# 123456jack/decision-making-and-path-planning

Measured on AMD Instinct MI355X. Metric: planning ticks/sec (batched scenes), 512x512 grid, higher is better.
Workload: dtype f64; 1 GPU; BASELINE configs[1]: 1024 scenes/GPU, 512x512 grid, 64 static obstacles; scenes_per_gpu=1024, global_scenes=1024, grid=512, obstacles=64, parallelism=scene-sharded x1, RCCL scatter/gather outside the timed region, algorithmic_bytes_per_tick=276644

## Files before the change

### decision-making-and-path-planning_amd/csrc/dmpp_hip.hip

```cpp
#include <hip/hip_runtime.h>
#include <cstddef>
#include <cstdio>
#include <cstring>
#include <cmath>
#include <string>
#include <cstdlib>
#include <vector>
#include <new>
#include <algorithm>
#include "../../include/dmpp_planner.h"
#include "kernels_r.hpp"
#include "kernels_a.hpp"
#include "kernels_rt.hpp"
#include "kernels_ep.hpp"
#include "kernels_es.hpp"
#include "kernels_g.hpp"
#include "kernels_sc.hpp"
#include "kernels_el.hpp"
#include "kernels_f.hpp"
#include "kernels_t.hpp"
#include "kernels_op.hpp"
#include "search_budget.hpp"

namespace {
// ... 1992 lines not shown
    if (h->rec_last.tick != T) {
        { int r = join_all(h); if (r) return r; }
        hipEvent_t e = get_sync_event(h);
        if (!e) return fail(PP_ERR_HIP, "event creation failed");
        HIP_TRY(hipEventRecord(e, h->stream));
        TickRec rec = { T, h->in_cur, e, nullptr };
        h->inflight.push_back(rec); h->rec_last = rec;
    }
    const TickRec& R = h->rec_last;
    if (h->done_tick[slot] != T) { h->done_tick[slot] = T; h->done_g[slot].forget(); h->done_p[slot].forget(); }
    const bool want_plan = plan || result || show;
    PendingFetch f{};
    f.tick = T; f.slot = slot; f.n = (size_t)n; f.ev_front = R.ev_front; f.ev_tail = R.ev_tail;
    if (want_plan) { f.plan_dst = plan; f.res_dst = result; f.show_dst = show; f.plan_src = h->d_plan; f.plan_set = h->plan_cur; }
    if (grid) { f.grid_dst = grid; f.grid_src = h->d_gout[h->gout_set]; f.grid_set = h->gout_set; }
    bool joined = false;
    for (PendingFetch& g : h->fetches) if (g.tick == T) {
        if (want_plan && !g.plan_dst && !g.res_dst && !g.show_dst) { g.plan_dst = f.plan_dst; g.res_dst = f.res_dst; g.show_dst = f.show_dst; g.plan_src = f.plan_src; g.plan_set = f.plan_set; g.plan_issued = false; joined = true; }
        if (grid && !g.grid_dst) { g.grid_dst = f.grid_dst; g.grid_src = f.grid_src; g.grid_set = f.grid_set; g.grid_issued = false; joined = true; }
    }
    if (!joined) h->fetches.push_back(f);
    { int r = pump_fetches(h); if (r) return r; }
    if (tick_id) *tick_id = T;
    return PP_OK;
}

int pp_fetch_async(pp_handle h, PlanOut* plan, GridOut* grid, long long* tick_id) { return fetch_async(h, plan, nullptr, nullptr, grid, tick_id); }
int pp_fetch_published_async(pp_handle h, PlanningOut* result, PlanningStatus* show, GridOut* grid, long long* tick_id)
{ return fetch_async(h, nullptr, result, show, grid, tick_id); }

long long pp_tick_id(pp_handle h) { return h ? h->tick_seq : -1; }

int pp_wait_tick(pp_handle h, long long tick_id, int* n_poisoned)
{
    if (!h) return fail(PP_ERR_ARG, "null handle");
    if (n_poisoned) *n_poisoned = 0;
    if (tick_id <= 0 || tick_id > h->tick_seq) return fail(PP_ERR_ARG, "pp_wait_tick: no such tick");
    const int slot = (int)(tick_id % kDone);
    if (!h->streaming || h->done_tick[slot] != tick_id)
        return fail(PP_ERR_ARG, "pp_wait_tick: no pp_fetch_async was issued for that tick (or more than " + std::to_string(kDone) + " ticks ago)");
    HIP_TRY(hipSetDevice(h->device));
    { int r = flush_group(h); if (r) return r; }
    { int r = pump_fetches(h, tick_id); if (r) return r; }
    PP_TRY(h->done_p[slot].host_wait());
    PP_TRY(h->done_g[slot].host_wait());
    const int bad = (int)reinterpret_cast<volatile int32_t*>(h->h_bad.get())[slot];
    if (n_poisoned) *n_poisoned = bad;
    if (bad) return fail(PP_ERR_ARG, "tick " + std::to_string(tick_id) + ": " + std::to_string(bad) + " scene(s) of its update had a slice outside its pool (or a road / lane outside the map) and ran with empty inputs");
    return PP_OK;
}

int pp_tick_io(pp_handle h, PpSceneIo* io)
{
    if (!h || !io) return fail(PP_ERR_ARG, "null argument");
    if (h->n_scenes != 1) return fail(PP_ERR_STATE, "pp_tick_io moves ONE resident scene (pp_set_scenes with n_scenes = 1 comes first: its lane pool stays)");
    if ((io->want & PP_IO_WANT_GRID) && !h->cfg.grid_stage) return fail(PP_ERR_STATE, "PP_IO_WANT_GRID: the handle's configuration has the grid stage off");
    HIP_TRY(hipSetDevice(h->device));
    const int max_obs = std::min(PP_IO_MAX_OBS, h->caps.max_obs_total), max_ref = std::min(DMPP_MAX_REFPATH, h->caps.max_ref_pts_total);
    { int r = flush_group(h); if (r) return r; }
    PP_TRY(h->score.ego.wait(h->stream));
    h->in_staged = -1; h->rollout.staged_by_advance = false;
    hipLaunchKernelGGL(dmpp::k_io_in, dim3(1), dim3(dmpp::kBlock), 0, h->stream, io, max_obs, max_ref, h->n_lane_pts, h->d_in, h->d_state, h->d_obs, h->d_ref);
    HIP_TRY(hipGetLastError());
    h->n_obs_total = std::min(std::max((int)io->n_obs, 0), max_obs); h->have_motion = false;
    h->n_ref_pts = std::max(h->n_ref_pts, max_ref);
    note_current_set(h);
    { int r = pp_plan_tick(h); if (r) return r; }
    if (h->last_piped) { int r = join_all(h); if (r) return r; }
    hipLaunchKernelGGL(dmpp::k_io_out, dim3(1), dim3(dmpp::kBlock), 0, h->stream, io, (int)io->want, h->d_plan, h->d_state,
                       h->cfg.grid_stage ? h->d_gout[h->gout_set] : nullptr, h->d_dec_ref);
    HIP_TRY(hipGetLastError());
    HIP_TRY(hipStreamSynchronize(h->stream));
    if (reinterpret_cast<volatile int32_t*>(&io->status)[0]) return fail(PP_ERR_ARG, "pp_tick_io: a lane slice of io->in lies outside the resident lane pool (the scene ran with empty lanes)");
    return PP_OK;
}

#ifdef DMPP_DEBUG_SEARCH
int pp_debug_score_counters(int* out8, int reset)
{
    HIP_TRY(hipMemcpyFromSymbol(out8, HIP_SYMBOL(dmpp::g_dbg_score), 8 * sizeof(int)));
    if (reset) { int z[8] = { 0 }; HIP_TRY(hipMemcpyToSymbol(HIP_SYMBOL(dmpp::g_dbg_score), z, sizeof(z))); }
    return PP_OK;
}
#endif

void* pp_host_alloc(size_t bytes)
{
    void* p = nullptr;
    if (hipHostMalloc(&p, bytes ? bytes : 1, hipHostMallocDefault) != hipSuccess) { (void)hipGetLastError(); g_err = "hipHostMalloc failed"; return nullptr; }
    return p;
}
void pp_host_free(void* p) { if (p) (void)hipHostFree(p); }
int pp_host_register(void* p, size_t bytes)
{
    if (!p || !bytes) return fail(PP_ERR_ARG, "null argument");
    HIP_TRY(hipHostRegister(p, bytes, hipHostRegisterDefault));
    return PP_OK;
}
int pp_host_unregister(void* p) { if (!p) return PP_OK; HIP_TRY(hipHostUnregister(p)); return PP_OK; }

static int need_scratch(pp_handle h, size_t bytes)
{
    if (bytes <= h->d_scratch.capacity()) return PP_OK;
    HIP_TRY(hipStreamSynchronize(h->stream));
    return h->d_scratch.reserve(bytes);
}
static size_t al256(size_t v) { return (v + 255) & ~(size_t)255; }

int pp_search_obstacle_batch(pp_handle h, int nq, const GlobalPoint2D* paths, const int32_t* path_off, const ObPoint* obs,
                             const int32_t* obs_off, const double* lat_lo, const double* lat_hi, Path_Obs* out)
{
    if (!h || !paths || !path_off || !obs_off || !lat_lo || !lat_hi || !out) return fail(PP_ERR_ARG, "null argument");
    if (nq <= 0) return PP_OK;
    HIP_TRY(hipSetDevice(h->device));
    const int np = path_off[nq], no = obs_off[nq];
    for (int q = 0; q < nq; q++) if (path_off[q + 1] - path_off[q] > dmpp::kSoMaxPts) return fail(PP_ERR_CAPACITY, "a path longer than 2048 points");
    size_t o_paths = 0, o_poff = o_paths + al256((size_t)np * sizeof(GlobalPoint2D)), o_obs = o_poff + al256((size_t)(nq + 1) * 4),
           o_ooff = o_obs + al256((size_t)no * sizeof(ObPoint)), o_lo = o_ooff + al256((size_t)(nq + 1) * 4),
           o_hi = o_lo + al256((size_t)nq * 8), o_out = o_hi + al256((size_t)nq * 8), total = o_out + al256((size_t)nq * sizeof(Path_Obs));
    int r = need_scratch(h, total); if (r) return r;
    char* d = (char*)h->d_scratch;
    if (np) HIP_TRY(hipMemcpyAsync(d + o_paths, paths, (size_t)np * sizeof(GlobalPoint2D), hipMemcpyDefault, h->stream));
    HIP_TRY(hipMemcpyAsync(d + o_poff, path_off, (size_t)(nq + 1) * 4, hipMemcpyDefault, h->stream));
    if (no && obs) HIP_TRY(hipMemcpyAsync(d + o_obs, obs, (size_t)no * sizeof(ObPoint), hipMemcpyDefault, h->stream));
    HIP_TRY(hipMemcpyAsync(d + o_ooff, obs_off, (size_t)(nq + 1) * 4, hipMemcpyDefault, h->stream));
    HIP_TRY(hipMemcpyAsync(d + o_lo, lat_lo, (size_t)nq * 8, hipMemcpyDefault, h->stream));
    HIP_TRY(hipMemcpyAsync(d + o_hi, lat_hi, (size_t)nq * 8, hipMemcpyDefault, h->stream));
    hipLaunchKernelGGL(dmpp::k_search_obstacle_batch, dim3(nq), dim3(DMPP_WAVE), 0, h->stream, h->cfg, nq,
                       (const GlobalPoint2D*)(d + o_paths), (const int32_t*)(d + o_poff), (const ObPoint*)(d + o_obs),
                       (const int32_t*)(d + o_ooff), (const double*)(d + o_lo), (const double*)(d + o_hi), (Path_Obs*)(d + o_out));
    HIP_TRY(hipGetLastError());
    HIP_TRY(hipMemcpyAsync(out, d + o_out, (size_t)nq * sizeof(Path_Obs), hipMemcpyDefault, h->stream));
    HIP_TRY(hipStreamSynchronize(h->stream));
    return PP_OK;
}

int pp_geom_batch(pp_handle h, int op, int n, const GlobalPoint2D* a, const GlobalPoint2D* b, const GlobalPoint2D* c3, double* out)
{
    if (!h || !a || !out || op < 0 || op > 5) return fail(PP_ERR_ARG, "bad argument");
    if (((op <= 1 || op == 3) && !b) || (op == 0 && !c3)) return fail(PP_ERR_ARG, "missing operand");
    if (n <= 0) return PP_OK;
    HIP_TRY(hipSetDevice(h->device));
    const size_t pb = al256((size_t)n * sizeof(GlobalPoint2D));
    int r = need_scratch(h, 3 * pb + al256((size_t)n * 8)); if (r) return r;
    char* d = (char*)h->d_scratch;
    HIP_TRY(hipMemcpyAsync(d, a, (size_t)n * sizeof(GlobalPoint2D), hipMemcpyDefault, h->stream));
    if (b) HIP_TRY(hipMemcpyAsync(d + pb, b, (size_t)n * sizeof(GlobalPoint2D), hipMemcpyDefault, h->stream));
    if (c3) HIP_TRY(hipMemcpyAsync(d + 2 * pb, c3, (size_t)n * sizeof(GlobalPoint2D), hipMemcpyDefault, h->stream));
    hipLaunchKernelGGL(dmpp::k_geom_batch, dim3((n + 255) / 256), dim3(256), 0, h->stream, h->cfg, op, n, (const GlobalPoint2D*)d,
                       (const GlobalPoint2D*)(d + pb), (const GlobalPoint2D*)(d + 2 * pb), (double*)(d + 3 * pb));
    HIP_TRY(hipGetLastError());
    HIP_TRY(hipMemcpyAsync(out, d + 3 * pb, (size_t)n * 8, hipMemcpyDefault, h->stream));
    HIP_TRY(hipStreamSynchronize(h->stream));
    return PP_OK;
}

int pp_scalar_stage(pp_handle h, int op, const double* in, int n_in, const GlobalPoint2D* last_Bpoints, double* out, int n_out)
{
    if (!h || !in || !out || op < 0 || op > 2 || n_in < 1 || n_in > 8 || n_out < 1 || n_out > 4) return fail(PP_ERR_ARG, "bad argument");
    if (op == 2 && !last_Bpoints) return fail(PP_ERR_ARG, "CalculateRadius needs the 200 path points");
    HIP_TRY(hipSetDevice(h->device));
    int r = need_scratch(h, 4096 + DMPP_PATH_POINTS * sizeof(GlobalPoint2D)); if (r) return r;
    char* d = (char*)h->d_scratch;
    HIP_TRY(hipMemcpyAsync(d, in, (size_t)n_in * 8, hipMemcpyDefault, h->stream));
    if (op == 2) HIP_TRY(hipMemcpyAsync(d + 4096, last_Bpoints, DMPP_PATH_POINTS * sizeof(GlobalPoint2D), hipMemcpyDefault, h->stream));
    hipLaunchKernelGGL(dmpp::k_scalar_stage, dim3(1), dim3(64), 0, h->stream, h->cfg, op, (const double*)d,
// ... 147 lines not shown
```

### decision-making-and-path-planning_amd/csrc/kernels_g.hpp

```cpp
#pragma once
#include "dev_geom.hpp"
#include "kernels_s.hpp"
#include "kernels_score.hpp"

namespace dmpp {

constexpr int kOrderBlock = 1024;
__global__ void __launch_bounds__(kOrderBlock)
k_order(int n_items, const int32_t* __restrict__ cost, int32_t* __restrict__ perm)
{
    __shared__ int cnt[kOrderClasses], base[kOrderClasses];
    const int tid = threadIdx.x;
    cnt[tid] = 0;
    __syncthreads();
    for (int s = tid; s < n_items; s += kOrderBlock) atomicAdd(&cnt[kOrderClasses - 1 - min(max(cost[s], 0), kOrderClasses - 1)], 1);
    __syncthreads();
    base[tid] = cnt[tid];
    __syncthreads();
    for (int d = 1; d < kOrderClasses; d <<= 1) {
        const int v = tid >= d ? base[tid - d] : 0;
        __syncthreads();
        base[tid] += v;
        __syncthreads();
    }
    base[tid] -= cnt[tid];
    __syncthreads();
    for (int s = tid; s < n_items; s += kOrderBlock)
        perm[atomicAdd(&base[kOrderClasses - 1 - min(max(cost[s], 0), kOrderClasses - 1)], 1)] = s;
}

template <int NW>
__global__ void __launch_bounds__(NW * DMPP_WAVE)
k_score(PlannerConfig c, int n_items, const TickGroup g, int32_t* __restrict__ need_dev, int32_t* __restrict__ need_host)
{
    extern __shared__ __align__(16) unsigned char smem_raw[];
    ScoreShared<NW>& sh = *reinterpret_cast<ScoreShared<NW>*>(smem_raw);
    const int w = blockIdx.x;
    if (w == 0 && threadIdx.x == 0 && need_dev) {
        const int32_t v = need_dev[0];
        need_dev[0] = 0;
        need_dev[1] = 0;
        if (need_host) *need_host = v;
    }
    if (w >= n_items) return;
#ifdef DMPP_SCORE_PRIO
    __builtin_amdgcn_s_setprio(DMPP_SCORE_PRIO);
#endif
    const int slot = w / g.n, scene = w - slot * g.n;
    const SceneIn& si = g.in[scene];
    GridOut& go = g.gout[slot * g.gout_stride + scene];
    score_body<NW>(c, si, g.obs_now + slot * g.obs_stride + si.obs_off, si.obs_n, g.paths + slot * g.path_stride + (size_t)scene * c.max_path, go, go.status, go.path_len, sh);
}

}
```

### decision-making-and-path-planning_amd/csrc/kernels_score.hpp

```cpp
#pragma once
#include "dev_geom.hpp"

namespace dmpp {

constexpr int kBoxWaves = 4;
constexpr int kTailRounds = 4, kTailFirst = 190;
template <int NW> constexpr bool kPackTail = NW <= 4;
template <int NW> constexpr int kTailWaves = NW <= 4 ? NW : 1;
static_assert(DMPP_PATH_POINTS - 192 == 8 && kTailFirst == 190 && kTailRounds * 8 <= DMPP_WAVE, "packed fourth pass: lane 8 c + j = point 192 + j of candidate c");
static_assert(DMPP_PATH_POINTS <= kBoxWaves * DMPP_WAVE && DMPP_MAX_LATTICE <= 32, "score_body: lane layouts");
constexpr int kMaxRelObs = 128;
constexpr int kBucketN = 12, kBucketCap = 12, kBucketMinObs = 8;
#ifdef DMPP_DEBUG_SEARCH
__device__ int g_dbg_score[8];
#endif
template <int NW>
struct ScoreShared {
    GlobalPoint2D cand[NW][DMPP_PATH_POINTS];
    GlobalPoint2D pts[DMPP_PATH_POINTS];
    double cum[DMPP_PATH_POINTS];
    double rx[kMaxRelObs], ry[kMaxRelObs], rr[kMaxRelObs], rt2[kMaxRelObs];
    Bezier bz[DMPP_MAX_LATTICE];
    double trig[4];
    double bb[4];
    GlobalPoint2D T;
    double cost[DMPP_MAX_LATTICE];
    int box[4][4];
    GlobalPoint2D tail[kTailWaves<NW>][kTailRounds][DMPP_PATH_POINTS - kTailFirst];
    int best, n_rel;
    int bcnt[kBucketN * kBucketN];
    unsigned char bent[kBucketN * kBucketN][kBucketCap];
};

__device__ __forceinline__ double wave_tree_sum(double acc)
{
#pragma unroll
    for (int sft = 32; sft >= 1; sft >>= 1) acc += shfl_xor_f64(acc, sft);
    return acc;
}

template <int NW>
__device__ __forceinline__ void score_body(const PlannerConfig& c, const SceneIn& si, const ObPoint* __restrict__ gobs, int m,
                                           const int32_t* __restrict__ path, GridOut& go, int status, int path_len, ScoreShared<NW>& sh)
{
    constexpr int kThreads = NW * DMPP_WAVE;
    const int tid = threadIdx.x, wave = tid >> 6, lane = tid & 63;
    const int W = c.grid_w;
    const GlobalPoint3D ego = si.loc.globalpoint;
    const bool have_path = (status == DMPP_G_FOUND) && path_len >= 1;
    const int nl = min(c.n_lattice, DMPP_MAX_LATTICE - 1);
    const int nc = nl + (have_path ? 1 : 0);
    const double half_w = 0.5 * c.Vehicle_Width;
    int a = 0;
    if (have_path) {
        a = min(path_len - 1, c.lookahead_cells);
        if (a > DMPP_PATH_POINTS - 1) a = DMPP_PATH_POINTS - 1;
        int cx0 = 0x7fffffff, cx1 = -1, cy0 = 0x7fffffff, cy1 = -1;
        for (int i = tid; i <= a; i += kThreads) {
            const int pc = path[i];
            const int px = pc % W, py = pc / W;
            sh.pts[i].x = si.grid_origin.x + ((double)px + 0.5) * c.cell;
            sh.pts[i].y = si.grid_origin.y + ((double)py + 0.5) * c.cell;
            cx0 = min(cx0, px); cx1 = max(cx1, px); cy0 = min(cy0, py); cy1 = max(cy1, py);
        }
        if (wave < kBoxWaves) {
#pragma unroll
            for (int sft = 32; sft >= 1; sft >>= 1) {
                cx0 = min(cx0, __shfl_xor(cx0, sft, 64)); cx1 = max(cx1, __shfl_xor(cx1, sft, 64));
                cy0 = min(cy0, __shfl_xor(cy0, sft, 64)); cy1 = max(cy1, __shfl_xor(cy1, sft, 64));
            }
            if (lane == 0) { sh.box[wave][0] = cx0; sh.box[wave][1] = cx1; sh.box[wave][2] = cy0; sh.box[wave][3] = cy1; }
        }
    }
    if (wave == NW - 1) {
        GlobalPoint2D T; double thT;
        if (have_path) {
            const int a0 = max(a - 4, 0);
            const int pa = path[a], p0 = path[a0];
            T.x = si.grid_origin.x + ((double)(pa % W) + 0.5) * c.cell;
            T.y = si.grid_origin.y + ((double)(pa / W) + 0.5) * c.cell;
            if (a0 == a) thT = ego.dir;
            else {
                GlobalPoint2D P0 = { si.grid_origin.x + ((double)(p0 % W) + 0.5) * c.cell, si.grid_origin.y + ((double)(p0 / W) + 0.5) * c.cell };
                thT = GetRoadAngle(c, P0, T);
            }
        } else {
            T = si.goal;
            GlobalPoint2D e2 = { ego.x, ego.y };
            thT = GetRoadAngle(c, e2, si.goal);
        }
        const double ang = (lane == 0 ? ego.dir : thT) * c.PI / 180;
        double sv, cv;
        sincos(ang, &sv, &cv);
        if (lane == 0) { sh.trig[0] = cv; sh.trig[1] = sv; sh.T = T; }
        if (lane == 1) { sh.trig[2] = cv; sh.trig[3] = sv; }
    }
    __syncthreads();
    if (have_path && wave == 0) wave_cumlen(sh.pts, a + 1, sh.cum, lane);
    if (wave == NW - 1) {
        double X0 = __builtin_inf(), X1 = -__builtin_inf(), Y0 = __builtin_inf(), Y1 = -__builtin_inf();
        if (lane < nl) {
            const double c0 = sh.trig[0], s0 = sh.trig[1], cs = sh.trig[2], sn = sh.trig[3];
            const GlobalPoint2D T = sh.T;
            const double off = (double)(lane - (nl - 1) / 2) * c.lattice_step;
            Bezier bz;
            bz.x0 = ego.x; bz.y0 = ego.y; bz.x3 = T.x + off * sn; bz.y3 = T.y + off * (-cs);
            const double dx = bz.x3 - bz.x0, dy = bz.y3 - bz.y0;
            const double d = sqrt(dx * dx + dy * dy) / 3;
            bz.x1 = bz.x0 + d * c0; bz.y1 = bz.y0 + d * s0;
            bz.x2 = bz.x3 - d * cs; bz.y2 = bz.y3 - d * sn;
            sh.bz[lane] = bz;
            X0 = fmin(fmin(bz.x0, bz.x1), fmin(bz.x2, bz.x3)); X1 = fmax(fmax(bz.x0, bz.x1), fmax(bz.x2, bz.x3));
            Y0 = fmin(fmin(bz.y0, bz.y1), fmin(bz.y2, bz.y3)); Y1 = fmax(fmax(bz.y0, bz.y1), fmax(bz.y2, bz.y3));
        }
#pragma unroll
        for (int sft = 16; sft >= 1; sft >>= 1) {
            X0 = fmin(X0, shfl_xor_f64(X0, sft)); X1 = fmax(X1, shfl_xor_f64(X1, sft));
            Y0 = fmin(Y0, shfl_xor_f64(Y0, sft)); Y1 = fmax(Y1, shfl_xor_f64(Y1, sft));
        }
        if (lane == 0) { sh.bb[0] = X0; sh.bb[1] = X1; sh.bb[2] = Y0; sh.bb[3] = Y1; sh.n_rel = 0; }
    }
    __syncthreads();
    double X0 = sh.bb[0], X1 = sh.bb[1], Y0 = sh.bb[2], Y1 = sh.bb[3];
    if (have_path) {
        int cx0 = 0x7fffffff, cx1 = -1, cy0 = 0x7fffffff, cy1 = -1;
        for (int w = 0; w < (NW < kBoxWaves ? NW : kBoxWaves); w++) {
            cx0 = min(cx0, sh.box[w][0]); cx1 = max(cx1, sh.box[w][1]); cy0 = min(cy0, sh.box[w][2]); cy1 = max(cy1, sh.box[w][3]);
        }
        X0 = fmin(X0, si.grid_origin.x + ((double)cx0 - 0.5) * c.cell); X1 = fmax(X1, si.grid_origin.x + ((double)cx1 + 1.5) * c.cell);
        Y0 = fmin(Y0, si.grid_origin.y + ((double)cy0 - 0.5) * c.cell); Y1 = fmax(Y1, si.grid_origin.y + ((double)cy1 + 1.5) * c.cell);
    }
    for (int j = tid; j < m; j += kThreads) {
        const ObPoint o = gobs[j];
        const double thr = (double)o.radius + half_w + c.d_safe;
        if (o.x >= X0 - thr && o.x <= X1 + thr && o.y >= Y0 - thr && o.y <= Y1 + thr) {
            const int q = atomicAdd(&sh.n_rel, 1);
            if (q < kMaxRelObs) { sh.rx[q] = o.x; sh.ry[q] = o.y; sh.rr[q] = (double)o.radius; sh.rt2[q] = thr * thr; }
        }
    }
    __syncthreads();
    const bool culled = sh.n_rel <= kMaxRelObs;
    const int n_rel = culled ? sh.n_rel : m;
    const double inv_bx = (X1 > X0) ? (double)kBucketN / (X1 - X0) : 0.0, inv_by = (Y1 > Y0) ? (double)kBucketN / (Y1 - Y0) : 0.0;
    auto bucket_x = [&](double v) { return clampi((int)floor((v - X0) * inv_bx), 0, kBucketN - 1); };
    auto bucket_y = [&](double v) { return clampi((int)floor((v - Y0) * inv_by), 0, kBucketN - 1); };
    const bool bucketed = culled ? n_rel >= kBucketMinObs : m <= 256;
    if (bucketed) {
        for (int i = tid; i < kBucketN * kBucketN; i += kThreads) sh.bcnt[i] = 0;
        __syncthreads();
        for (int j = tid; j < n_rel; j += kThreads) {
            double ox, oy, r;
            if (culled) { ox = sh.rx[j]; oy = sh.ry[j]; r = sh.rr[j]; }
            else { const ObPoint o = gobs[j]; ox = o.x; oy = o.y; r = (double)o.radius; }
            const double thr = (r + half_w + c.d_safe) * (1.0 + 1e-9) + 1e-9;
            if (!(ox >= X0 - thr && ox <= X1 + thr && oy >= Y0 - thr && oy <= Y1 + thr)) continue;
            const int bx0 = bucket_x(ox - thr), bx1 = bucket_x(ox + thr), by0 = bucket_y(oy - thr), by1 = bucket_y(oy + thr);
            for (int by = by0; by <= by1; by++)
                for (int bx = bx0; bx <= bx1; bx++) {
                    const int b = by * kBucketN + bx;
                    const int q = atomicAdd(&sh.bcnt[b], 1);
                    if (q < kBucketCap) sh.bent[b][q] = (unsigned char)j;
                }
        }
        __syncthreads();
    }
#ifdef DMPP_DEBUG_SEARCH
    if (tid == 0) {
        atomicAdd(&g_dbg_score[0], 1); atomicAdd(&g_dbg_score[1], sh.n_rel); atomicAdd(&g_dbg_score[2], bucketed ? 1 : 0);
        { int ov = 0; if (bucketed) for (int i = 0; i < kBucketN * kBucketN; i++) ov += sh.bcnt[i] > kBucketCap; atomicAdd(&g_dbg_score[3], ov); }
        atomicAdd(&g_dbg_score[4], culled ? 0 : 1);
        atomicMax(&g_dbg_score[5], sh.n_rel);
    }
#endif
    GlobalPoint2D* cand = sh.cand[wave];
    double wb0[4], wb1[4], wb2[4], wb3[4];
#pragma unroll
    for (int q = 0; q < 4; q++) {
        const int i = lane + 64 * q;
        const double t = (double)i / (double)(DMPP_PATH_POINTS - 1), u = 1 - t;
        wb0[q] = u * u * u; wb1[q] = 3 * u * u * t; wb2[q] = 3 * u * t * t; wb3[q] = t * t * t;
    }
    const double kk2_fenced = 0.001 * 0.001;
    auto point_terms = [&](const GlobalPoint2D* cnd, int i, const GlobalPoint2D p, double& pen, double& kk2, bool& hit) {
        double clear = __builtin_inf();
        int nb = 0, b = 0;
        if (bucketed) { b = bucket_y(p.y) * kBucketN + bucket_x(p.x); nb = sh.bcnt[b]; }
        if (bucketed && nb <= kBucketCap) {
            for (int e = 0; e < nb; e++) {
                const int j = sh.bent[b][e];
                double ox, oy, r, t2;
                if (culled) { ox = sh.rx[j]; oy = sh.ry[j]; r = sh.rr[j]; t2 = sh.rt2[j]; }
                else { ox = gobs[j].x; oy = gobs[j].y; r = (double)gobs[j].radius; const double thr = r + half_w + c.d_safe; t2 = thr * thr; }
                const double dx = p.x - ox, dy = p.y - oy;
                const double d2 = dx * dx + dy * dy;
                if (d2 > t2) continue;
                const double v = sqrt(d2) - r;
                if (v < clear) clear = v;
            }
        } else if (__builtin_expect(culled, 1)) {
            for (int j = 0; j < n_rel; j++) {
                const double dx = p.x - sh.rx[j], dy = p.y - sh.ry[j];
                const double d2 = dx * dx + dy * dy;
                if (d2 > sh.rt2[j]) continue;
                const double v = sqrt(d2) - sh.rr[j];
                if (v < clear) clear = v;
            }
        } else {
            for (int j = 0; j < m; j++) {
                const double dx = p.x - gobs[j].x, dy = p.y - gobs[j].y;
                const double d2 = dx * dx + dy * dy;
                const double thr = (double)gobs[j].radius + half_w + c.d_safe;
                if (d2 > thr * thr) continue;
                const double v = sqrt(d2) - (double)gobs[j].radius;
                if (v < clear) clear = v;
            }
        }
        clear = clear - half_w;
        hit = false;
        if (clear <= 0) { pen = 1000.0; hit = true; }
        else if (clear < c.d_safe) { const double qq = (c.d_safe - clear) / c.d_safe; pen = qq * qq; }
        else pen = 0;
        kk2 = 0;
        if (i >= 1 && i <= DMPP_PATH_POINTS - 2) {
            const GlobalPoint2D pa = cnd[i - 1], pf = cnd[i + 1];
            const double d1 = (pa.x - p.x) * (pa.x - p.x) + (pa.y - p.y) * (pa.y - p.y);
            const double d2 = (p.x - pf.x) * (p.x - pf.x) + (p.y - pf.y) * (p.y - pf.y);
            const double d3 = (pa.x - pf.x) * (pa.x - pf.x) + (pa.y - pf.y) * (pa.y - pf.y);
            const double den2 = 4 * d1 * d2, num = d1 + d2 - d3;
            const double diff = den2 - num * num, fence = kk2_fenced * den2;
            kk2 = kk2_fenced;
            if (den2 > 0) {
                if (__builtin_expect(fabs(diff - fence) <= 1e-6 * fence, 0)) {
                    const double dis1 = sqrt(d1), dis2 = sqrt(d2), dis3 = sqrt(d3);
                    const double den = 2 * dis1 * dis2;
                    if (den > 0) {
                        const double cosA = (dis1 * dis1 + dis2 * dis2 - dis3 * dis3) / den;
                        const double sinA = sqrt(1 - cosA * cosA);
                        if (sinA >= 0.001) { const double R = 0.5 * dis3 / sinA; const double kq = 1 / R; kk2 = kq * kq; }
                    }
                } else if (diff > fence) kk2 = diff / (d1 * d2 * d3);
            }
        }
    };
    auto publish = [&](int k, double off, double pen_acc, double k2_acc, int first_hit) {
        const double col = wave_tree_sum(pen_acc), curv = wave_tree_sum(k2_acc);
#pragma unroll
        for (int sft = 32; sft >= 1; sft >>= 1) first_hit = min(first_hit, __shfl_xor(first_hit, sft, 64));
        const double prog = (first_hit == DMPP_PATH_POINTS) ? 0.0 : (double)(DMPP_PATH_POINTS - first_hit) / (double)DMPP_PATH_POINTS;
        const double cost = c.w_col * col + c.w_curv * curv + c.w_prog * prog + c.w_off * fabs(off);
        if (lane == 0) { go.cand_col[k] = col; go.cand_curv[k] = curv; go.cand_prog[k] = prog; go.cand_cost[k] = cost; sh.cost[k] = cost; }
    };
    const int left = nc % NW, n_whole = (4 * left <= NW) ? nc - left : nc;
    auto whole_candidate = [&](int k, int n_pass, double& off, double& pen_acc, double& k2_acc, int& first_hit, GlobalPoint2D* tail) {
        off = 0;
        if (k < nl) {
            const Bezier bz = sh.bz[k];
            off = (double)(k - (nl - 1) / 2) * c.lattice_step;
#pragma unroll
            for (int q = 0; q < 4; q++) {
                GlobalPoint2D P;
                P.x = wb0[q] * bz.x0 + wb1[q] * bz.x1 + wb2[q] * bz.x2 + wb3[q] * bz.x3;
                P.y = wb0[q] * bz.y0 + wb1[q] * bz.y1 + wb2[q] * bz.y2 + wb3[q] * bz.y3;
                if (lane + 64 * q < DMPP_PATH_POINTS) cand[lane + 64 * q] = P;
            }
        } else {
#pragma nounroll
            for (int q = 0; q < 4; q++)
                if (lane + 64 * q < DMPP_PATH_POINTS) cand[lane + 64 * q] = mean_point(c, sh.pts, sh.cum, a + 1, lane + 64 * q, DMPP_PATH_POINTS);
        }
        wave_sync();
        if (tail && lane < DMPP_PATH_POINTS - kTailFirst) tail[lane] = cand[kTailFirst + lane];
        pen_acc = 0; k2_acc = 0; first_hit = DMPP_PATH_POINTS;
#pragma nounroll
        for (int q = 0; q < n_pass; q++) {
            const int i = lane + 64 * q;
            if (i < DMPP_PATH_POINTS) {
                double pen, kk2; bool hit;
                point_terms(cand, i, cand[i], pen, kk2, hit);
                pen_acc += pen; k2_acc += kk2;
                if (hit && i < first_hit) first_hit = i;
            }
        }
        wave_sync();
    };
    const int rounds = (n_whole - wave + NW - 1) / NW;
    const bool pack_tail = kPackTail<NW> && (n_whole + NW - 1) / NW >= 2 && (n_whole + NW - 1) / NW <= kTailRounds;
    {
        double accP[kTailRounds], accK[kTailRounds], accOff[kTailRounds]; int accH[kTailRounds];
#pragma unroll
        for (int t = 0; t < kTailRounds; t++) { accP[t] = 0; accK[t] = 0; accOff[t] = 0; accH[t] = DMPP_PATH_POINTS; }
#pragma nounroll
        for (int ci = 0; ci < rounds; ci++) {
            const int k = wave + ci * NW;
            double off, pen_acc, k2_acc; int first_hit;
            whole_candidate(k, pack_tail ? 3 : 4, off, pen_acc, k2_acc, first_hit, pack_tail ? &sh.tail[wave % kTailWaves<NW>][ci][0] : nullptr);
            if (!pack_tail) publish(k, off, pen_acc, k2_acc, first_hit);
            else {
#pragma unroll
                for (int t = 0; t < kTailRounds; t++) if (t == ci) { accP[t] = pen_acc; accK[t] = k2_acc; accOff[t] = off; accH[t] = first_hit; }
            }
        }
        if (pack_tail) {
            {
                const int cl = lane >> 3, i = 192 + (lane & 7);
                double pen = 0, kk2 = 0; bool hit = false;
                if (cl < rounds) {
                    const GlobalPoint2D* cnd = &sh.tail[wave % kTailWaves<NW>][cl][0] - kTailFirst;
                    point_terms(cnd, i, cnd[i], pen, kk2, hit);
                }
                const int hv = hit ? i : DMPP_PATH_POINTS;
#pragma unroll
                for (int ci = 0; ci < kTailRounds; ci++) {
                    const double vp = shfl_f64(pen, 8 * ci + (lane & 7)), vk = shfl_f64(kk2, 8 * ci + (lane & 7));
                    const int vh = __shfl(hv, 8 * ci + (lane & 7), 64);
                    if (ci < rounds && lane < DMPP_PATH_POINTS - 192) { accP[ci] += vp; accK[ci] += vk; accH[ci] = min(accH[ci], vh); }
                }
            }
#pragma unroll
            for (int ci = 0; ci < kTailRounds; ci++) if (ci < rounds) publish(wave + ci * NW, accOff[ci], accP[ci], accK[ci], accH[ci]);
        }
    }
    if (n_whole < nc) {
        struct Part { double pen[DMPP_WAVE], k2[DMPP_WAVE]; int hit[DMPP_WAVE]; };
        static_assert(sizeof(Part) * NW <= sizeof(GlobalPoint2D) * DMPP_PATH_POINTS * (NW - NW / 4), "the partial sums live in the candidate arrays the left-over candidates do not use");
        Part* parts = reinterpret_cast<Part*>(&sh.cand[NW / 4][0]);
        __syncthreads();
        const bool mine = wave < 4 * left;
        const int j = wave >> 2, q = wave & 3, k = n_whole + j, i = lane + 64 * q;
        GlobalPoint2D p = { 0.0, 0.0 };
        if (mine) {
            if (k < nl) {
                const Bezier bz = sh.bz[k];
                const double b0 = q == 0 ? wb0[0] : q == 1 ? wb0[1] : q == 2 ? wb0[2] : wb0[3], b1 = q == 0 ? wb1[0] : q == 1 ? wb1[1] : q == 2 ? wb1[2] : wb1[3];
                const double b2 = q == 0 ? wb2[0] : q == 1 ? wb2[1] : q == 2 ? wb2[2] : wb2[3], b3 = q == 0 ? wb3[0] : q == 1 ? wb3[1] : q == 2 ? wb3[2] : wb3[3];
                p.x = b0 * bz.x0 + b1 * bz.x1 + b2 * bz.x2 + b3 * bz.x3;
                p.y = b0 * bz.y0 + b1 * bz.y1 + b2 * bz.y2 + b3 * bz.y3;
            } else p = mean_point(c, sh.pts, sh.cum, a + 1, min(i, DMPP_PATH_POINTS - 1), DMPP_PATH_POINTS);
            if (i < DMPP_PATH_POINTS) sh.cand[j][i] = p;
        }
        __syncthreads();
        if (mine) {
            double pen = 0, kk2 = 0; bool hit = false;
            if (i < DMPP_PATH_POINTS) point_terms(sh.cand[j], i, p, pen, kk2, hit);
            parts[wave].pen[lane] = pen; parts[wave].k2[lane] = kk2; parts[wave].hit[lane] = hit ? i : DMPP_PATH_POINTS;
        }
        __syncthreads();
        if (wave < left) {
            const int k2i = n_whole + wave;
            double pen_acc = 0, k2_acc = 0; int first_hit = DMPP_PATH_POINTS;
#pragma unroll
            for (int qq = 0; qq < 4; qq++) {
                if (lane + 64 * qq < DMPP_PATH_POINTS) {
                    const Part& pt = parts[wave * 4 + qq];
                    pen_acc += pt.pen[lane]; k2_acc += pt.k2[lane]; first_hit = min(first_hit, pt.hit[lane]);
                }
            }
            const double off2 = k2i < nl ? (double)(k2i - (nl - 1) / 2) * c.lattice_step : 0.0;
            publish(k2i, off2, pen_acc, k2_acc, first_hit);
        }
    }
    __syncthreads();
    if (tid == 0) {
        double best = 0; int bi = 0;
        for (int k = 0; k < nc; k++) if (k == 0 || sh.cost[k] < best) { best = sh.cost[k]; bi = k; }
        sh.best = bi; go.best_candidate = bi; go.n_candidates = nc;
        for (int k = nc; k < DMPP_MAX_LATTICE; k++) { go.cand_cost[k] = 0; go.cand_col[k] = 0; go.cand_curv[k] = 0; go.cand_prog[k] = 0; }
    }
    __syncthreads();
    {
        const int k = sh.best;
        if (tid < DMPP_PATH_POINTS) {
            GlobalPoint2D p = { 0.0, 0.0 };
            if (k < nl) {
                p = bezier_point(sh.bz[k], tid, DMPP_PATH_POINTS);
            } else if (nc > 0) p = mean_point(c, sh.pts, sh.cum, a + 1, tid, DMPP_PATH_POINTS);
            go.best_path[tid] = p;
        }
    }
}

}
```

Baseline: 5.908 million ticks/s.

## Pass score-kernel path neighbours via DPP lane shifts and shrink shared memory

Result: faster. 6.193 million ticks/s, median of 6 (+4.8%).

```diff
diff --git a/decision-making-and-path-planning_amd/csrc/dmpp_hip.hip b/decision-making-and-path-planning_amd/csrc/dmpp_hip.hip
--- a/decision-making-and-path-planning_amd/csrc/dmpp_hip.hip
+++ b/decision-making-and-path-planning_amd/csrc/dmpp_hip.hip
@@ -2098,6 +2098,13 @@
     if (reset) { int z[8] = { 0 }; HIP_TRY(hipMemcpyToSymbol(HIP_SYMBOL(dmpp::g_dbg_score), z, sizeof(z))); }
     return PP_OK;
 }
+int pp_debug_score_stamps(unsigned* out, int n_items)
+{
+    if (!out || n_items < 0 || n_items > dmpp::kDbgScoreItems) return fail(PP_ERR_ARG, "pp_debug_score_stamps: bad argument");
+    HIP_TRY(hipDeviceSynchronize());
+    HIP_TRY(hipMemcpyFromSymbol(out, HIP_SYMBOL(dmpp::g_dbg_score_ph), (size_t)n_items * dmpp::kDbgScorePhases * sizeof(unsigned)));
+    return PP_OK;
+}
 #endif
 
 void* pp_host_alloc(size_t bytes)
diff --git a/decision-making-and-path-planning_amd/csrc/kernels_g.hpp b/decision-making-and-path-planning_amd/csrc/kernels_g.hpp
--- a/decision-making-and-path-planning_amd/csrc/kernels_g.hpp
+++ b/decision-making-and-path-planning_amd/csrc/kernels_g.hpp
@@ -35,6 +35,12 @@
 {
     extern __shared__ __align__(16) unsigned char smem_raw[];
     ScoreShared<NW>& sh = *reinterpret_cast<ScoreShared<NW>*>(smem_raw);
+#ifdef DMPP_DEBUG_SEARCH
+    const long long dbg_t0 = clock64();
+#define SCORE_DBG_ARG , dbg_t0
+#else
+#define SCORE_DBG_ARG
+#endif
     const int w = blockIdx.x;
     if (w == 0 && threadIdx.x == 0 && need_dev) {
         const int32_t v = need_dev[0];
@@ -49,7 +55,7 @@
     const int slot = w / g.n, scene = w - slot * g.n;
     const SceneIn& si = g.in[scene];
     GridOut& go = g.gout[slot * g.gout_stride + scene];
-    score_body<NW>(c, si, g.obs_now + slot * g.obs_stride + si.obs_off, si.obs_n, g.paths + slot * g.path_stride + (size_t)scene * c.max_path, go, go.status, go.path_len, sh);
+    score_body<NW>(c, si, g.obs_now + slot * g.obs_stride + si.obs_off, si.obs_n, g.paths + slot * g.path_stride + (size_t)scene * c.max_path, go, go.status, go.path_len, sh SCORE_DBG_ARG);
 }
 
 }
diff --git a/decision-making-and-path-planning_amd/csrc/kernels_score.hpp b/decision-making-and-path-planning_amd/csrc/kernels_score.hpp
--- a/decision-making-and-path-planning_amd/csrc/kernels_score.hpp
+++ b/decision-making-and-path-planning_amd/csrc/kernels_score.hpp
@@ -4,33 +4,58 @@
 namespace dmpp {
 
 constexpr int kBoxWaves = 4;
-constexpr int kTailRounds = 4, kTailFirst = 190;
+constexpr int kTailRounds = 4;
 template <int NW> constexpr bool kPackTail = NW <= 4;
-template <int NW> constexpr int kTailWaves = NW <= 4 ? NW : 1;
-static_assert(DMPP_PATH_POINTS - 192 == 8 && kTailFirst == 190 && kTailRounds * 8 <= DMPP_WAVE, "packed fourth pass: lane 8 c + j = point 192 + j of candidate c");
+static_assert(DMPP_PATH_POINTS - 192 == 8 && kTailRounds * 8 <= DMPP_WAVE, "packed fourth pass: lane 8 c + j = point 192 + j of candidate c");
 static_assert(DMPP_PATH_POINTS <= kBoxWaves * DMPP_WAVE && DMPP_MAX_LATTICE <= 32, "score_body: lane layouts");
 constexpr int kMaxRelObs = 128;
 constexpr int kBucketN = 12, kBucketCap = 12, kBucketMinObs = 8;
 #ifdef DMPP_DEBUG_SEARCH
 __device__ int g_dbg_score[8];
+constexpr int kDbgScoreItems = 4096, kDbgScorePhases = 8;
+__device__ unsigned g_dbg_score_ph[kDbgScoreItems][kDbgScorePhases];
+#define SCORE_MARK(slot) { if (threadIdx.x == 0 && blockIdx.x < kDbgScoreItems) g_dbg_score_ph[blockIdx.x][slot] = (unsigned)(clock64() - dbg_t0); }
+#define SCORE_DBG_PARAM , long long dbg_t0
+#else
+#define SCORE_MARK(slot)
+#define SCORE_DBG_PARAM
 #endif
+struct ScoreLists {
+    double rx[kMaxRelObs], ry[kMaxRelObs], rr[kMaxRelObs], rt2[kMaxRelObs];
+    int bcnt[kBucketN * kBucketN];
+    unsigned char bent[kBucketN * kBucketN][kBucketCap];
+};
+struct ScorePart { double pen[DMPP_WAVE], k2[DMPP_WAVE]; int hit[DMPP_WAVE]; };
 template <int NW>
 struct ScoreShared {
-    GlobalPoint2D cand[NW][DMPP_PATH_POINTS];
     GlobalPoint2D pts[DMPP_PATH_POINTS];
     double cum[DMPP_PATH_POINTS];
-    double rx[kMaxRelObs], ry[kMaxRelObs], rr[kMaxRelObs], rt2[kMaxRelObs];
+    union { ScoreLists ls; ScorePart part[NW]; };
     Bezier bz[DMPP_MAX_LATTICE];
     double trig[4];
     double bb[4];
     GlobalPoint2D T;
     double cost[DMPP_MAX_LATTICE];
     int box[4][4];
-    GlobalPoint2D tail[kTailWaves<NW>][kTailRounds][DMPP_PATH_POINTS - kTailFirst];
     int best, n_rel;
-    int bcnt[kBucketN * kBucketN];
-    unsigned char bent[kBucketN * kBucketN][kBucketCap];
 };
+static_assert(sizeof(ScorePart) * 4 <= sizeof(ScoreLists), "k_score<4>: the partial sums of the left-over candidate fit over the obstacle lists and buckets");
+static_assert(sizeof(ScoreShared<4>) <= 11 * 1280, "k_score<4>: two workgroups per freed search slot at the configs[1] budget");
+
+__device__ __forceinline__ double lane_below_f64(double v)
+{
+    int lo = __double2loint(v), hi = __double2hiint(v);
+    lo = __builtin_amdgcn_update_dpp(lo, lo, 0x138, 0xf, 0xf, false);
+    hi = __builtin_amdgcn_update_dpp(hi, hi, 0x138, 0xf, 0xf, false);
+    return __hiloint2double(hi, lo);
+}
+__device__ __forceinline__ double lane_above_f64(double v)
+{
+    int lo = __double2loint(v), hi = __double2hiint(v);
+    lo = __builtin_amdgcn_update_dpp(lo, lo, 0x130, 0xf, 0xf, false);
+    hi = __builtin_amdgcn_update_dpp(hi, hi, 0x130, 0xf, 0xf, false);
+    return __hiloint2double(hi, lo);
+}
 
 __device__ __forceinline__ double wave_tree_sum(double acc)
 {
@@ -41,12 +66,19 @@
 
 template <int NW>
 __device__ __forceinline__ void score_body(const PlannerConfig& c, const SceneIn& si, const ObPoint* __restrict__ gobs, int m,
-                                           const int32_t* __restrict__ path, GridOut& go, int status, int path_len, ScoreShared<NW>& sh)
+                                           const int32_t* __restrict__ path, GridOut& go, int status, int path_len, ScoreShared<NW>& sh SCORE_DBG_PARAM)
 {
+    SCORE_MARK(0)
     constexpr int kThreads = NW * DMPP_WAVE;
     const int tid = threadIdx.x, wave = tid >> 6, lane = tid & 63;
     const int W = c.grid_w;
+    static_assert(DMPP_PATH_POINTS <= kThreads, "one cell of the path prefix per thread");
     const GlobalPoint3D ego = si.loc.globalpoint;
+    const GlobalPoint2D org = si.grid_origin, goal = si.goal;
+    int pc_mine = 0;
+    if (tid <= min(c.lookahead_cells, DMPP_PATH_POINTS - 1) && tid < c.max_path) pc_mine = path[tid];
+    ObPoint o_mine; o_mine.x = 0; o_mine.y = 0; o_mine.radius = 0;
+    if (tid < m) o_mine = gobs[tid];
     const bool have_path = (status == DMPP_G_FOUND) && path_len >= 1;
     const int nl = min(c.n_lattice, DMPP_MAX_LATTICE - 1);
     const int nc = nl + (have_path ? 1 : 0);
@@ -56,12 +88,11 @@
         a = min(path_len - 1, c.lookahead_cells);
         if (a > DMPP_PATH_POINTS - 1) a = DMPP_PATH_POINTS - 1;
         int cx0 = 0x7fffffff, cx1 = -1, cy0 = 0x7fffffff, cy1 = -1;
-        for (int i = tid; i <= a; i += kThreads) {
-            const int pc = path[i];
-            const int px = pc % W, py = pc / W;
-            sh.pts[i].x = si.grid_origin.x + ((double)px + 0.5) * c.cell;
-            sh.pts[i].y = si.grid_origin.y + ((double)py + 0.5) * c.cell;
-            cx0 = min(cx0, px); cx1 = max(cx1, px); cy0 = min(cy0, py); cy1 = max(cy1, py);
+        if (tid <= a) {
+            const int px = pc_mine % W, py = pc_mine / W;
+            sh.pts[tid].x = org.x + ((double)px + 0.5) * c.cell;
+            sh.pts[tid].y = org.y + ((double)py + 0.5) * c.cell;
+            cx0 = px; cx1 = px; cy0 = py; cy1 = py;
         }
         if (wave < kBoxWaves) {
 #pragma unroll
@@ -72,32 +103,27 @@
             if (lane == 0) { sh.box[wave][0] = cx0; sh.box[wave][1] = cx1; sh.box[wave][2] = cy0; sh.box[wave][3] = cy1; }
         }
     }
+    SCORE_MARK(1)
+    __syncthreads();
+    if (have_path && wave == 0) wave_cumlen(sh.pts, a + 1, sh.cum, lane);
     if (wave == NW - 1) {
         GlobalPoint2D T; double thT;
         if (have_path) {
             const int a0 = max(a - 4, 0);
-            const int pa = path[a], p0 = path[a0];
-            T.x = si.grid_origin.x + ((double)(pa % W) + 0.5) * c.cell;
-            T.y = si.grid_origin.y + ((double)(pa / W) + 0.5) * c.cell;
+            T = sh.pts[a];
             if (a0 == a) thT = ego.dir;
-            else {
-                GlobalPoint2D P0 = { si.grid_origin.x + ((double)(p0 % W) + 0.5) * c.cell, si.grid_origin.y + ((double)(p0 / W) + 0.5) * c.cell };
-                thT = GetRoadAngle(c, P0, T);
-            }
+            else thT = GetRoadAngle(c, sh.pts[a0], T);
         } else {
-            T = si.goal;
+            T = goal;
             GlobalPoint2D e2 = { ego.x, ego.y };
-            thT = GetRoadAngle(c, e2, si.goal);
+            thT = GetRoadAngle(c, e2, goal);
         }
         const double ang = (lane == 0 ? ego.dir : thT) * c.PI / 180;
         double sv, cv;
         sincos(ang, &sv, &cv);
         if (lane == 0) { sh.trig[0] = cv; sh.trig[1] = sv; sh.T = T; }
         if (lane == 1) { sh.trig[2] = cv; sh.trig[3] = sv; }
-    }
-    __syncthreads();
-    if (have_path && wave == 0) wave_cumlen(sh.pts, a + 1, sh.cum, lane);
-    if (wave == NW - 1) {
+        wave_sync();
         double X0 = __builtin_inf(), X1 = -__builtin_inf(), Y0 = __builtin_inf(), Y1 = -__builtin_inf();
         if (lane < nl) {
             const double c0 = sh.trig[0], s0 = sh.trig[1], cs = sh.trig[2], sn = sh.trig[3];
@@ -121,21 +147,22 @@
         if (lane == 0) { sh.bb[0] = X0; sh.bb[1] = X1; sh.bb[2] = Y0; sh.bb[3] = Y1; sh.n_rel = 0; }
     }
     __syncthreads();
+    SCORE_MARK(2)
     double X0 = sh.bb[0], X1 = sh.bb[1], Y0 = sh.bb[2], Y1 = sh.bb[3];
     if (have_path) {
         int cx0 = 0x7fffffff, cx1 = -1, cy0 = 0x7fffffff, cy1 = -1;
         for (int w = 0; w < (NW < kBoxWaves ? NW : kBoxWaves); w++) {
             cx0 = min(cx0, sh.box[w][0]); cx1 = max(cx1, sh.box[w][1]); cy0 = min(cy0, sh.box[w][2]); cy1 = max(cy1, sh.box[w][3]);
         }
-        X0 = fmin(X0, si.grid_origin.x + ((double)cx0 - 0.5) * c.cell); X1 = fmax(X1, si.grid_origin.x + ((double)cx1 + 1.5) * c.cell);
-        Y0 = fmin(Y0, si.grid_origin.y + ((double)cy0 - 0.5) * c.cell); Y1 = fmax(Y1, si.grid_origin.y + ((double)cy1 + 1.5) * c.cell);
+        X0 = fmin(X0, org.x + ((double)cx0 - 0.5) * c.cell); X1 = fmax(X1, org.x + ((double)cx1 + 1.5) * c.cell);
+        Y0 = fmin(Y0, org.y + ((double)cy0 - 0.5) * c.cell); Y1 = fmax(Y1, org.y + ((double)cy1 + 1.5) * c.cell);
     }
     for (int j = tid; j < m; j += kThreads) {
-        const ObPoint o = gobs[j];
+        const ObPoint o = j == tid ? o_mine : gobs[j];
         const double thr = (double)o.radius + half_w + c.d_safe;
         if (o.x >= X0 - thr && o.x <= X1 + thr && o.y >= Y0 - thr && o.y <= Y1 + thr) {
             const int q = atomicAdd(&sh.n_rel, 1);
-            if (q < kMaxRelObs) { sh.rx[q] = o.x; sh.ry[q] = o.y; sh.rr[q] = (double)o.radius; sh.rt2[q] = thr * thr; }
+            if (q < kMaxRelObs) { sh.ls.rx[q] = o.x; sh.ls.ry[q] = o.y; sh.ls.rr[q] = (double)o.radius; sh.ls.rt2[q] = thr * thr; }
         }
     }
     __syncthreads();
@@ -146,11 +173,11 @@
     auto bucket_y = [&](double v) { return clampi((int)floor((v - Y0) * inv_by), 0, kBucketN - 1); };
     const bool bucketed = culled ? n_rel >= kBucketMinObs : m <= 256;
     if (bucketed) {
-        for (int i = tid; i < kBucketN * kBucketN; i += kThreads) sh.bcnt[i] = 0;
+        for (int i = tid; i < kBucketN * kBucketN; i += kThreads) sh.ls.bcnt[i] = 0;
         __syncthreads();
         for (int j = tid; j < n_rel; j += kThreads) {
             double ox, oy, r;
-            if (culled) { ox = sh.rx[j]; oy = sh.ry[j]; r = sh.rr[j]; }
+            if (culled) { ox = sh.ls.rx[j]; oy = sh.ls.ry[j]; r = sh.ls.rr[j]; }
             else { const ObPoint o = gobs[j]; ox = o.x; oy = o.y; r = (double)o.radius; }
             const double thr = (r + half_w + c.d_safe) * (1.0 + 1e-9) + 1e-9;
             if (!(ox >= X0 - thr && ox <= X1 + thr && oy >= Y0 - thr && oy <= Y1 + thr)) continue;
@@ -158,8 +185,8 @@
             for (int by = by0; by <= by1; by++)
                 for (int bx = bx0; bx <= bx1; bx++) {
                     const int b = by * kBucketN + bx;
-                    const int q = atomicAdd(&sh.bcnt[b], 1);
-                    if (q < kBucketCap) sh.bent[b][q] = (unsigned char)j;
+                    const int q = atomicAdd(&sh.ls.bcnt[b], 1);
+                    if (q < kBucketCap) sh.ls.bent[b][q] = (unsigned char)j;
                 }
         }
         __syncthreads();
@@ -167,29 +194,28 @@
 #ifdef DMPP_DEBUG_SEARCH
     if (tid == 0) {
         atomicAdd(&g_dbg_score[0], 1); atomicAdd(&g_dbg_score[1], sh.n_rel); atomicAdd(&g_dbg_score[2], bucketed ? 1 : 0);
-        { int ov = 0; if (bucketed) for (int i = 0; i < kBucketN * kBucketN; i++) ov += sh.bcnt[i] > kBucketCap; atomicAdd(&g_dbg_score[3], ov); }
+        { int ov = 0; if (bucketed) for (int i = 0; i < kBucketN * kBucketN; i++) ov += sh.ls.bcnt[i] > kBucketCap; atomicAdd(&g_dbg_score[3], ov); }
         atomicAdd(&g_dbg_score[4], culled ? 0 : 1);
         atomicMax(&g_dbg_score[5], sh.n_rel);
     }
 #endif
-    GlobalPoint2D* cand = sh.cand[wave];
-    double wb0[4], wb1[4], wb2[4], wb3[4];
-#pragma unroll
-    for (int q = 0; q < 4; q++) {
-        const int i = lane + 64 * q;
-        const double t = (double)i / (double)(DMPP_PATH_POINTS - 1), u = 1 - t;
-        wb0[q] = u * u * u; wb1[q] = 3 * u * u * t; wb2[q] = 3 * u * t * t; wb3[q] = t * t * t;
-    }
+    SCORE_MARK(3)
+    auto cand_point = [&](int k, int i) -> GlobalPoint2D {
+        if (k < nl) return bezier_point(sh.bz[k], i, DMPP_PATH_POINTS);
+        return mean_point(c, sh.pts, sh.cum, a + 1, clampi(i, 0, DMPP_PATH_POINTS - 1), DMPP_PATH_POINTS);
+    };
+    auto from_lane_below = [&](const GlobalPoint2D p) -> GlobalPoint2D { GlobalPoint2D r; r.x = lane_below_f64(p.x); r.y = lane_below_f64(p.y); return r; };
+    auto from_lane_above = [&](const GlobalPoint2D p) -> GlobalPoint2D { GlobalPoint2D r; r.x = lane_above_f64(p.x); r.y = lane_above_f64(p.y); return r; };
     const double kk2_fenced = 0.001 * 0.001;
-    auto point_terms = [&](const GlobalPoint2D* cnd, int i, const GlobalPoint2D p, double& pen, double& kk2, bool& hit) {
+    auto point_terms = [&](int i, const GlobalPoint2D p, const GlobalPoint2D pa, const GlobalPoint2D pf, double& pen, double& kk2, bool& hit) {
         double clear = __builtin_inf();
         int nb = 0, b = 0;
-        if (bucketed) { b = bucket_y(p.y) * kBucketN + bucket_x(p.x); nb = sh.bcnt[b]; }
+        if (bucketed) { b = bucket_y(p.y) * kBucketN + bucket_x(p.x); nb = sh.ls.bcnt[b]; }
         if (bucketed && nb <= kBucketCap) {
             for (int e = 0; e < nb; e++) {
-                const int j = sh.bent[b][e];
+                const int j = sh.ls.bent[b][e];
                 double ox, oy, r, t2;
-                if (culled) { ox = sh.rx[j]; oy = sh.ry[j]; r = sh.rr[j]; t2 = sh.rt2[j]; }
+                if (culled) { ox = sh.ls.rx[j]; oy = sh.ls.ry[j]; r = sh.ls.rr[j]; t2 = sh.ls.rt2[j]; }
                 else { ox = gobs[j].x; oy = gobs[j].y; r = (double)gobs[j].radius; const double thr = r + half_w + c.d_safe; t2 = thr * thr; }
                 const double dx = p.x - ox, dy = p.y - oy;
                 const double d2 = dx * dx + dy * dy;
@@ -199,10 +225,10 @@
             }
         } else if (__builtin_expect(culled, 1)) {
             for (int j = 0; j < n_rel; j++) {
-                const double dx = p.x - sh.rx[j], dy = p.y - sh.ry[j];
+                const double dx = p.x - sh.ls.rx[j], dy = p.y - sh.ls.ry[j];
                 const double d2 = dx * dx + dy * dy;
-                if (d2 > sh.rt2[j]) continue;
-                const double v = sqrt(d2) - sh.rr[j];
+                if (d2 > sh.ls.rt2[j]) continue;
+                const double v = sqrt(d2) - sh.ls.rr[j];
                 if (v < clear) clear = v;
             }
         } else {
@@ -222,7 +248,6 @@
         else pen = 0;
         kk2 = 0;
         if (i >= 1 && i <= DMPP_PATH_POINTS - 2) {
-            const GlobalPoint2D pa = cnd[i - 1], pf = cnd[i + 1];
             const double d1 = (pa.x - p.x) * (pa.x - p.x) + (pa.y - p.y) * (pa.y - p.y);
             const double d2 = (p.x - pf.x) * (p.x - pf.x) + (p.y - pf.y) * (p.y - pf.y);
             const double d3 = (pa.x - pf.x) * (pa.x - pf.x) + (pa.y - pf.y) * (pa.y - pf.y);
@@ -251,37 +276,29 @@
         if (lane == 0) { go.cand_col[k] = col; go.cand_curv[k] = curv; go.cand_prog[k] = prog; go.cand_cost[k] = cost; sh.cost[k] = cost; }
     };
     const int left = nc % NW, n_whole = (4 * left <= NW) ? nc - left : nc;
-    auto whole_candidate = [&](int k, int n_pass, double& off, double& pen_acc, double& k2_acc, int& first_hit, GlobalPoint2D* tail) {
+    auto whole_candidate = [&](int k, int n_pass, double& off, double& pen_acc, double& k2_acc, int& first_hit) {
         off = 0;
-        if (k < nl) {
-            const Bezier bz = sh.bz[k];
-            off = (double)(k - (nl - 1) / 2) * c.lattice_step;
-#pragma unroll
-            for (int q = 0; q < 4; q++) {
-                GlobalPoint2D P;
-                P.x = wb0[q] * bz.x0 + wb1[q] * bz.x1 + wb2[q] * bz.x2 + wb3[q] * bz.x3;
-                P.y = wb0[q] * bz.y0 + wb1[q] * bz.y1 + wb2[q] * bz.y2 + wb3[q] * bz.y3;
-                if (lane + 64 * q < DMPP_PATH_POINTS) cand[lane + 64 * q] = P;
-            }
-        } else {
-#pragma nounroll
-            for (int q = 0; q < 4; q++)
-                if (lane + 64 * q < DMPP_PATH_POINTS) cand[lane + 64 * q] = mean_point(c, sh.pts, sh.cum, a + 1, lane + 64 * q, DMPP_PATH_POINTS);
-        }
-        wave_sync();
-        if (tail && lane < DMPP_PATH_POINTS - kTailFirst) tail[lane] = cand[kTailFirst + lane];
+        if (k < nl) off = (double)(k - (nl - 1) / 2) * c.lattice_step;
         pen_acc = 0; k2_acc = 0; first_hit = DMPP_PATH_POINTS;
+        GlobalPoint2D P = cand_point(k, lane), below = P;
 #pragma nounroll
         for (int q = 0; q < n_pass; q++) {
             const int i = lane + 64 * q;
+            GlobalPoint2D N = P;
+            if (64 * (q + 1) < DMPP_PATH_POINTS) N = cand_point(k, i + 64);
+            GlobalPoint2D pa = from_lane_below(P), pf = from_lane_above(P);
+            const GlobalPoint2D above = { readlane_f64(N.x, 0), readlane_f64(N.y, 0) };
+            if (lane == 0) pa = below;
+            if (lane == DMPP_WAVE - 1) pf = above;
             if (i < DMPP_PATH_POINTS) {
                 double pen, kk2; bool hit;
-                point_terms(cand, i, cand[i], pen, kk2, hit);
+                point_terms(i, P, pa, pf, pen, kk2, hit);
                 pen_acc += pen; k2_acc += kk2;
                 if (hit && i < first_hit) first_hit = i;
             }
-        }
-        wave_sync();
+            below.x = readlane_f64(P.x, DMPP_WAVE - 1); below.y = readlane_f64(P.y, DMPP_WAVE - 1);
+            P = N;
+        }
     };
     const int rounds = (n_whole - wave + NW - 1) / NW;
     const bool pack_tail = kPackTail<NW> && (n_whole + NW - 1) / NW >= 2 && (n_whole + NW - 1) / NW <= kTailRounds;
@@ -293,21 +310,24 @@
         for (int ci = 0; ci < rounds; ci++) {
             const int k = wave + ci * NW;
             double off, pen_acc, k2_acc; int first_hit;
-            whole_candidate(k, pack_tail ? 3 : 4, off, pen_acc, k2_acc, first_hit, pack_tail ? &sh.tail[wave % kTailWaves<NW>][ci][0] : nullptr);
+            whole_candidate(k, pack_tail ? 3 : 4, off, pen_acc, k2_acc, first_hit);
             if (!pack_tail) publish(k, off, pen_acc, k2_acc, first_hit);
             else {
 #pragma unroll
                 for (int t = 0; t < kTailRounds; t++) if (t == ci) { accP[t] = pen_acc; accK[t] = k2_acc; accOff[t] = off; accH[t] = first_hit; }
             }
         }
+        SCORE_MARK(4)
         if (pack_tail) {
             {
                 const int cl = lane >> 3, i = 192 + (lane & 7);
+                const int kc = wave + (cl < rounds ? cl : 0) * NW;
                 double pen = 0, kk2 = 0; bool hit = false;
-                if (cl < rounds) {
-                    const GlobalPoint2D* cnd = &sh.tail[wave % kTailWaves<NW>][cl][0] - kTailFirst;
-                    point_terms(cnd, i, cnd[i], pen, kk2, hit);
-                }
+                const GlobalPoint2D p = cand_point(kc, i), p191 = cand_point(kc, 191);
+                GlobalPoint2D pa = from_lane_below(p);
+                const GlobalPoint2D pf = from_lane_above(p);
+                if ((lane & 7) == 0) pa = p191;
+                if (cl < rounds) point_terms(i, p, pa, pf, pen, kk2, hit);
                 const int hv = hit ? i : DMPP_PATH_POINTS;
 #pragma unroll
                 for (int ci = 0; ci < kTailRounds; ci++) {
@@ -320,30 +340,20 @@
             for (int ci = 0; ci < kTailRounds; ci++) if (ci < rounds) publish(wave + ci * NW, accOff[ci], accP[ci], accK[ci], accH[ci]);
         }
     }
+    SCORE_MARK(5)
     if (n_whole < nc) {
-        struct Part { double pen[DMPP_WAVE], k2[DMPP_WAVE]; int hit[DMPP_WAVE]; };
-        static_assert(sizeof(Part) * NW <= sizeof(GlobalPoint2D) * DMPP_PATH_POINTS * (NW - NW / 4), "the partial sums live in the candidate arrays the left-over candidates do not use");
-        Part* parts = reinterpret_cast<Part*>(&sh.cand[NW / 4][0]);
-        __syncthreads();
         const bool mine = wave < 4 * left;
         const int j = wave >> 2, q = wave & 3, k = n_whole + j, i = lane + 64 * q;
-        GlobalPoint2D p = { 0.0, 0.0 };
+        double pen = 0, kk2 = 0; bool hit = false;
         if (mine) {
-            if (k < nl) {
-                const Bezier bz = sh.bz[k];
-                const double b0 = q == 0 ? wb0[0] : q == 1 ? wb0[1] : q == 2 ? wb0[2] : wb0[3], b1 = q == 0 ? wb1[0] : q == 1 ? wb1[1] : q == 2 ? wb1[2] : wb1[3];
-                const double b2 = q == 0 ? wb2[0] : q == 1 ? wb2[1] : q == 2 ? wb2[2] : wb2[3], b3 = q == 0 ? wb3[0] : q == 1 ? wb3[1] : q == 2 ? wb3[2] : wb3[3];
-                p.x = b0 * bz.x0 + b1 * bz.x1 + b2 * bz.x2 + b3 * bz.x3;
-                p.y = b0 * bz.y0 + b1 * bz.y1 + b2 * bz.y2 + b3 * bz.y3;
-            } else p = mean_point(c, sh.pts, sh.cum, a + 1, min(i, DMPP_PATH_POINTS - 1), DMPP_PATH_POINTS);
-            if (i < DMPP_PATH_POINTS) sh.cand[j][i] = p;
+            const GlobalPoint2D p = cand_point(k, i), e = cand_point(k, lane == 0 ? i - 1 : i + 1);
+            GlobalPoint2D pa = from_lane_below(p), pf = from_lane_above(p);
+            if (lane == 0) pa = e;
+            if (lane == DMPP_WAVE - 1) pf = e;
+            if (i < DMPP_PATH_POINTS) point_terms(i, p, pa, pf, pen, kk2, hit);
         }
         __syncthreads();
-        if (mine) {
-            double pen = 0, kk2 = 0; bool hit = false;
-            if (i < DMPP_PATH_POINTS) point_terms(sh.cand[j], i, p, pen, kk2, hit);
-            parts[wave].pen[lane] = pen; parts[wave].k2[lane] = kk2; parts[wave].hit[lane] = hit ? i : DMPP_PATH_POINTS;
-        }
+        if (mine) { sh.part[wave].pen[lane] = pen; sh.part[wave].k2[lane] = kk2; sh.part[wave].hit[lane] = hit ? i : DMPP_PATH_POINTS; }
         __syncthreads();
         if (wave < left) {
             const int k2i = n_whole + wave;
@@ -351,7 +361,7 @@
 #pragma unroll
             for (int qq = 0; qq < 4; qq++) {
                 if (lane + 64 * qq < DMPP_PATH_POINTS) {
-                    const Part& pt = parts[wave * 4 + qq];
+                    const ScorePart& pt = sh.part[wave * 4 + qq];
                     pen_acc += pt.pen[lane]; k2_acc += pt.k2[lane]; first_hit = min(first_hit, pt.hit[lane]);
                 }
             }
@@ -360,6 +370,7 @@
         }
     }
     __syncthreads();
+    SCORE_MARK(6)
     if (tid == 0) {
         double best = 0; int bi = 0;
         for (int k = 0; k < nc; k++) if (k == 0 || sh.cost[k] < best) { best = sh.cost[k]; bi = k; }
@@ -377,6 +388,7 @@
             go.best_path[tid] = p;
         }
     }
-}
-
-}
+    SCORE_MARK(7)
+}
+
+}
```
